# CTPLab/Tera-MIND

Measured on AMD Instinct MI355X. Metric: denoising steps/sec on 64x64x(2 stains x 2 z) patches (interior patch-steps/s), higher is better.
Workload: dtype f32; 1 GPU; configs[1]: b=32 images x 1 interior 64x64 patch (P=1, 128 padded + 32 collage patches/step), rna_slc=4, rna_num=229, stain=all, DDPM T=50 schedule, f32, mode A (pad+patchify -> UNet -> DDPM update); parallelism=dp1 (independent patch batches)

## Files before the change

### include/teramind_hip.h

```cpp
#ifndef TERAMIND_HIP_H
#define TERAMIND_HIP_H

#include <stddef.h>
#include <stdint.h>

#ifdef __cplusplus
extern "C" {
#endif

#define TM_ABI_VERSION 1

enum {
  TM_OK = 0,
  TM_ERR_ARG = -1,
  TM_ERR_STATE = -2,
  TM_ERR_KEY = -3,
  TM_ERR_HIP = -4,
  TM_ERR_WORKSPACE = -5
};

enum { TM_DTYPE_F32 = 0, TM_DTYPE_BF16 = 1, TM_DTYPE_F16 = 2 };
enum { TM_SAMPLE_DDPM = 0, TM_SAMPLE_DDIM = 1 };

typedef struct tm_config {
// ... 138 lines not shown
  double total_ms;
  double nominal_flops;
  double executed_flops;
  double alg_bytes;
} tm_prof_stats;
int tm_profile_enable(tm_model* m, int on);
int tm_profile_collect(tm_model* m, tm_prof_stats* out);


int tm_op_to_cb8(const void* x_ncdhw, void* y_cb8, int N, int C, int Z, int H, int W, void* stream);
int tm_op_from_cb8(const void* x_cb8, void* y_ncdhw, int N, int C, int Z, int H, int W, void* stream);

int tm_op_conv_mfma(const void* x_cb8, const void* w_host, const void* bias_host, void* y_cb8,
                    int N, int Cin, int Cout, int Z, int S, int ksize, int zmode, int up2,
                    int tile_variant, void* stream);
int tm_op_conv_mfma_res(const void* x_cb8, const void* w_host, const void* bias_host, void* y_cb8, const void* res_cb8,
                        int res_half, int N, int Cin, int Cout, int Z, int S, int ksize, int zmode, int up2,
                        int tile_variant, void* stream);

int tm_op_conv_zpair_fused_f32(const void* x_cb8, const void* w_host, const void* bias_host, const void* norm_w_host,
                               const void* scale_host, const void* shift_host, const void* res_cb8, void* a2_out,
                               void* h1_out, void* a2_sep_out, int N, int Cin, int Cout, int Z, int S, int per_image,
                               int tile_variant, void* stream);

int tm_op_conv_ups_pair_f32(const void* x_cb8, const void* w_host, const void* bias_host, void* y_cb8, int N, int Cin,
                            int Cout, int Z, int S, int tile_variant, void* stream);

int tm_op_conv_xpair_f32(const void* x_cb8, const void* w_host, const void* bias_host, void* y_cb8, const void* res_cb8,
                         int res_half, int N, int Cin, int Cout, int Z, int S, int tile_variant, void* stream);
int tm_op_conv_pad1_time_f32(const void* x_cb8, const void* w_host, const void* bias_host, void* y_cb8, int N, int Cin,
                             int Cout, int S, int form, int tile_variant, int iters, float* ms_out, void* stream);

int tm_op_conv1_f32(const void* x_cb8, const void* w_host, const void* bias_host, void* y_cb8, const void* res_cb8,
                    const void* gate_cb8, int x_cbtot, int x_cb0, int gate_cbtot, int gate_cb0, int gate_half, int gelu,
                    int tile_variant, int N, int Cin, int Cout, int Z, int S, int* form_out, void* stream);
int tm_conv1_form(long vox, int ntile, int tile_variant);

int tm_conv_frag_addrs(int kernel, int half, int tw, int what, int wave, int p, int ky, int kx, int sub, int* out64);

int tm_op_conv27_bf16(const void* x_cb8, const void* w_host, const void* bias_host, void* y_cb8,
                      int N, int Cin, int Cout, int S, int dtype, int waves, const void* res_h16, void* y_h16,
                      int ups, int res_half, void* stream);
int tm_op_conv27_h16_z(const void* x_cb8, const void* w_host, const void* bias_host, void* y_cb8,
                       int N, int Cin, int Cout, int S, int dtype, int waves, const void* res_h16, void* y_h16,
                       int ups, int res_half, int Z, void* stream);

// ... 135 lines not shown
```

### tera-mind_amd/_lib.py

```python
import ctypes as C
import os

_HERE = os.path.dirname(os.path.abspath(__file__))
LIB_PATH = os.environ.get("TM_LIB_PATH") or os.path.join(_HERE, "csrc", "libteramind_hip.so")

c_void_p, c_int, c_size_t, c_char_p, c_float = C.c_void_p, C.c_int, C.c_size_t, C.c_char_p, C.c_float
c_i64_p = C.POINTER(C.c_int64)


class TmConfig(C.Structure):
    _fields_ = [("patch_size", C.c_int32), ("rna_slc", C.c_int32), ("n_stain", C.c_int32),
                ("rna_num", C.c_int32), ("net_ch", C.c_int32), ("ch_mult", C.c_int32 * 4),
                ("embed_ch", C.c_int32), ("attn_res", C.c_int32), ("num_res_blocks", C.c_int32),
                ("vis_only", C.c_int32), ("dtype", C.c_int32)]


class TmStepCoefs(C.Structure):
    _fields_ = [("sqrt_recip_alphas_cumprod", c_float), ("sqrt_recipm1_alphas_cumprod", c_float),
                ("posterior_mean_coef1", c_float), ("posterior_mean_coef2", c_float),
                ("sigma", c_float), ("sqrt_alpha_bar_prev", c_float),
                ("sqrt_one_minus_alpha_bar_prev", c_float)]


class TmProfStats(C.Structure):
# ... 50 lines not shown
                                        C.c_int64, c_void_p, c_void_p]),
    "tm_blosc_frame_info": (c_int, [c_void_p, c_size_t, c_void_p]),
    "tm_blosc_decompress_dev": (c_int, [c_void_p, c_void_p, c_void_p, c_int, c_void_p, C.c_int64, c_void_p, c_void_p, c_void_p]),
    "tm_blosc_decompress_tiles": (c_int, [c_void_p, c_void_p, c_void_p, c_int, c_void_p, c_int] + [C.c_int64] * 3 + [c_void_p] * 3),
    "tm_u8_shrink2": (c_int, [c_void_p, c_int, c_int, C.c_int64, c_void_p, C.c_int64, c_void_p]),
    "tm_jpeg_encode_tiles": (c_int, [c_void_p, c_int, c_int, C.c_int64] + [c_int] * 3 + [c_void_p, C.c_int64] + [c_void_p] * 4),
    "tm_jpeg_tables": (c_int, [c_int, c_void_p, c_size_t, C.POINTER(c_size_t)]),
    "tm_ssim_planes": (c_int, [c_void_p, c_void_p] + [c_int] * 4 + [C.c_int64] * 4 + [C.POINTER(c_float), c_int, c_float, c_float, c_void_p, c_void_p]),
    "tm_avgpool2_pad": (c_int, [c_void_p] + [c_int] * 4 + [C.c_int64] * 2 + [c_void_p] + [C.c_int64] * 2 + [c_void_p]),
    "tm_profile_enable": (c_int, [c_void_p, c_int]),
    "tm_profile_collect": (c_int, [c_void_p, C.POINTER(TmProfStats)]),
    "tm_op_to_cb8": (c_int, [c_void_p, c_void_p, c_int, c_int, c_int, c_int, c_int, c_void_p]),
    "tm_op_from_cb8": (c_int, [c_void_p, c_void_p, c_int, c_int, c_int, c_int, c_int, c_void_p]),
    "tm_op_conv_mfma": (c_int, [c_void_p, c_void_p, c_void_p, c_void_p] + [c_int] * 9 + [c_void_p]),
    "tm_op_conv_mfma_res": (c_int, [c_void_p, c_void_p, c_void_p, c_void_p, c_void_p] + [c_int] * 10 + [c_void_p]),
    "tm_op_conv1_f32": (c_int, [c_void_p] * 6 + [c_int] * 12 + [C.POINTER(c_int), c_void_p]),
    "tm_conv1_form": (c_int, [C.c_long, c_int, c_int]),
    "tm_conv_frag_addrs": (c_int, [c_int] * 9 + [c_void_p]),
    "tm_op_conv27_bf16": (c_int, [c_void_p, c_void_p, c_void_p, c_void_p] + [c_int] * 6 + [c_void_p] * 2 + [c_int] * 2 + [c_void_p]),
    "tm_op_conv27_fused": (c_int, [c_void_p] * 7 + [c_int] * 7 + [c_void_p]),
    "tm_op_conv27_h16_z": (c_int, [c_void_p, c_void_p, c_void_p, c_void_p] + [c_int] * 6 + [c_void_p] * 2 + [c_int] * 3 + [c_void_p]),
    "tm_op_conv27_fused_z": (c_int, [c_void_p] * 7 + [c_int] * 8 + [c_void_p]),
    "tm_op_conv_zpair_fused_f32": (c_int, [c_void_p] * 10 + [c_int] * 7 + [c_void_p]),
    "tm_op_conv_ups_pair_f32": (c_int, [c_void_p] * 4 + [c_int] * 6 + [c_void_p]),
    "tm_op_conv_xpair_f32": (c_int, [c_void_p] * 5 + [c_int] * 7 + [c_void_p]),
    "tm_op_conv_pad1_time_f32": (c_int, [c_void_p] * 4 + [c_int] * 7 + [C.POINTER(c_float), c_void_p]),
    "tm_op_conv27_time":(c_int, [c_int] * 10 + [c_void_p, c_void_p]),
    "tm_op_conv1_bf16": (c_int, [c_void_p, c_void_p, c_void_p, c_void_p] + [c_int] * 8 + [c_void_p] * 4),
    "tm_op_conv1_h16_gate": (c_int, [c_void_p, c_void_p, c_void_p, c_void_p] + [c_int] * 8 + [c_void_p] * 3 + [c_int] * 3 + [c_void_p]),
    "tm_op_conv1_concat": (c_int, [c_void_p, c_void_p, c_void_p, c_int, c_void_p, c_void_p, c_void_p] + [c_int] * 8 + [c_void_p]),
    "tm_op_prep_h16": (c_int, [c_void_p] * 3 + [c_int] * 7 + [c_void_p, c_int, c_int, c_void_p, c_void_p, C.c_long] +
                       [c_int] * 4 + [c_void_p, c_void_p, c_int, c_void_p, c_void_p]),
    "tm_op_prep_f32": (c_int, [c_void_p] * 3 + [c_int] * 7 + [c_void_p, c_int, c_int, c_void_p, c_void_p, C.c_long] +
                       [c_int] * 4 + [c_void_p, c_void_p, c_int, c_void_p, c_void_p]),
    "tm_op_prep_form": (c_int, [c_void_p] * 3 + [c_int] * 9 + [c_void_p, c_int, c_int, c_int, c_void_p, c_void_p, C.c_long] +
                        [c_int] * 5 + [c_void_p, c_void_p, c_int, c_int, c_void_p, c_void_p]),
    "tm_op_stem": (c_int, [c_void_p] * 4 + [c_int] * 6 + [c_void_p]),
    "tm_op_head": (c_int, [c_void_p] * 4 + [c_int] * 6 + [c_void_p]),
    "tm_op_time_embed": (c_int, [c_void_p] * 7 + [c_int] * 3 + [c_void_p]),
    "tm_op_emb_all": (c_int, [c_void_p] * 4 + [c_int] * 3 + [c_void_p]),
    "tm_op_prep_train": (c_int, [c_void_p] * 5 + [c_float, c_int, c_void_p] + [c_int] * 4 + [c_void_p]),
    "tm_op_prep_bwd": (c_int, [c_void_p] * 6 + [c_float, c_int] + [c_void_p] * 4 + [c_int] * 4 + [c_void_p]),
    "tm_op_prep_train_rng": (c_int, [c_void_p] * 4 + [C.c_uint64, C.c_uint, c_float, c_int, c_void_p] + [c_int] * 4 + [c_void_p]),
    "tm_op_prep_bwd_rng": (c_int, [c_void_p] * 5 + [C.c_uint64, C.c_uint, c_float, c_int] + [c_void_p] * 4 + [c_int] * 4 + [c_void_p]),
    "tm_op_dropout_mask": (c_int, [C.c_uint64, C.c_uint, c_float, c_void_p] + [c_int] * 4 + [c_void_p]),
    "tm_op_conv_dgrad": (c_int, [c_void_p, c_void_p, c_void_p] + [c_int] * 6 + [c_void_p]),
# ... 63 lines not shown
```

### tera-mind_amd/csrc/tm_conv_pack.cpp

```cpp
#include "tm_conv_frag.h"
#include "tm_kernels.h"

#include <stdlib.h>
#include <string.h>

#include <vector>

namespace tmk {

int conv_form_taps(int form) {
  switch (form) {
    case CF_1X1: return 1;
    case CF_INPLANE: return 9;
    case CF_ZSKIP_UPS: case CF_PAIR_UPS: return 12;
    case CF_XPAIR: return 36;
    default: return 27;
  }
}
static bool form_ups(int form) { return form == CF_ZSKIP_UPS || form == CF_PAIR_UPS; }
size_t conv_pack_floats(int form, int Cout, int Cbi) {
  return (size_t)(form_ups(form) ? 4 : 1) * ((Cout + 63) / 64) * Cbi * conv_form_taps(form) * 512;
}
ConvW conv_w(int form, int Cout, int Cbi) {
  ConvW cw;
  cw.form = form; cw.Cout = Cout; cw.Cbi = Cbi; cw.taps = conv_form_taps(form); cw.ntile = (Cout + 63) / 64;
  return cw;
}

static bool switch_on(const char* name) {
  const char* v = getenv(name);
  return !(v && atoi(v) == 0);
}
int conv_pick_form(int ksize, int zmode, int Z, bool deep8, int role, bool* fuse_mid) {
  static const bool zpair_on = switch_on("TM_CONV_ZPAIR"), xpair_on = switch_on("TM_CONV_XPAIR"),
                    xmid_on = switch_on("TM_CONV_XPAIR_MID"), fuse_on = switch_on("TM_CONV_FUSE_MID");
  if (fuse_mid) *fuse_mid = false;
  if (ksize == 1) return CF_1X1;
  if (zmode == ZM_INPLANE) return CF_INPLANE;
  if (zmode == ZM_VALID) return CF_PLANES3;
  const bool pair = Z == 2 && zpair_on;
  if (zmode == ZM_UPS) return ((role & ROLE_OP_PAIR_UPS) || ((role & ROLE_RES) && pair)) ? CF_PAIR_UPS : CF_ZSKIP_UPS;
  if (Z != 2) return (Z == 1 && (role & ROLE_RES)) ? CF_INPLANE : CF_PLANES3;
  if ((role & ROLE_OP_XPAIR) && xpair_on) return CF_XPAIR;
  if (!pair) return CF_ZSKIP;
  const bool fuses = (role & ROLE_C1_64) && fuse_on;
  const bool xp = (role & ROLE_RES) && !(role & ROLE_DEEP) && xpair_on && deep8 && (!fuses || xmid_on);
  if (fuse_mid) *fuse_mid = fuses && !xp;
  return xp ? CF_XPAIR : CF_PAIR;
}

static void seg_counts(const int* seg_c, int nseg, int& Cin, int& Cbi) {
  Cin = Cbi = 0;
  for (int s = 0; s < nseg; ++s) { Cin += seg_c[s]; Cbi += (seg_c[s] + 7) / 8; }
}
static void pack_taps(const float* w, int Cout, const int* seg_c, int nseg, int taps, float* out, bool halves = false) {
  int Cin, Cbi;
  seg_counts(seg_c, nseg, Cin, Cbi);
  memset(out, 0, (size_t)((Cout + 63) / 64) * Cbi * taps * 512 * sizeof(float));
  int ci0 = 0, cb0 = 0;
  for (int s = 0; s < nseg; ++s) {
    for (int c = 0; c < seg_c[s]; ++c) {
      const int ci = ci0 + c;
      const int cb = cb0 + c / 8, c8 = c % 8;
      for (int co = 0; co < Cout; ++co) {
        const int nt = co / 64, col = co % 64;
        const float* src = w + ((size_t)co * Cin + ci) * taps;
        float* dst = out + (((size_t)nt * Cbi + cb) * taps) * 512 + (halves ? conv_w_off(col, c8) : col * 8 + c8);
        for (int t = 0; t < taps; ++t) dst[(size_t)t * 512] = src[t];
      }
    }
// ... 88 lines not shown
```

### tera-mind_amd/csrc/tm_device.h

```cpp
#pragma once
#include "tm_kernels.h"
#include <math.h>
#include <atomic>

namespace tmk {

typedef float f32x4 __attribute__((ext_vector_type(4)));
typedef float f32x16 __attribute__((ext_vector_type(16)));

#define TM_EPS 1e-6f

struct DevOnce {
  std::atomic<unsigned long long> done[2] = {{0ull}, {0ull}};
  static int dev() { int d = -1; return hipGetDevice(&d) == hipSuccess ? d : -1; }
  bool need() const {
    const int d = dev();
    if (d < 0 || d >= 128) return true;
    return !((done[d >> 6].load(std::memory_order_acquire) >> (d & 63)) & 1ull);
  }
  void mark() {
    const int d = dev();
    if (d >= 0 && d < 128) done[d >> 6].fetch_or(1ull << (d & 63), std::memory_order_release);
  }
};
// ... 137 lines not shown
        if (a.res) o = rv[g][mt] + o;
        if (a.y_h) {
          typedef TM_H16_T bf16x4_t __attribute__((ext_vector_type(4)));
          bf16x4_t ob;
#pragma unroll
          for (int j = 0; j < 4; ++j) ob[j] = (TM_H16_T)o[j];
          *(bf16x4_t*)(a.y_h + (long)on[mt] * a.yh_nstride + pl) = ob;
          continue;
        }
        float* yp = a.y + (long)on[mt] * a.y_nstride + pl;
        if (a.flags & EPI_UP2) {
          *(f32x4*)(yp) = o;
          *(f32x4*)(yp + 8) = o;
          *(f32x4*)(yp + (long)S_out * 8) = o;
          *(f32x4*)(yp + (long)S_out * 8 + 8) = o;
        } else {
          *(f32x4*)(yp) = o;
        }
      }
    }
  }
}

__device__ __forceinline__ void zpair_norm_epilogue(const ConvArgs& a, f32x16 (&o)[2][1], int h, int n, int ooff) {
  float s8[8];
#pragma unroll
  for (int ct = 0; ct < 2; ++ct)
#pragma unroll
    for (int g = 0; g < 4; ++g) {
      const f32x4 bv = *(const f32x4*)(a.bias + (ct * 4 + g) * 8 + 4 * h);
      float p[4];
#pragma unroll
      for (int j = 0; j < 4; ++j) {
        const float v = o[ct][0][4 * g + j] + bv[j];
        o[ct][0][4 * g + j] = v;
        p[j] = v * v;
        asm volatile("" : "+v"(p[j]));
      }
      const float lo = ((p[0] + p[1]) + p[2]) + p[3];
      const float lo_p = __shfl_xor(lo, 32, 64);
      s8[ct * 4 + g] = (((lo_p + p[0]) + p[1]) + p[2]) + p[3];
    }
  float red[4];
#pragma unroll
  for (int r = 0; r < 4; ++r) red[r] = s8[r] + s8[r + 4];
  const float t1 = ((red[0] + red[1]) + red[2]) + red[3];
  const float t0 = __shfl_xor(t1, 32, 64);
  const float t = h ? t1 : t0;
  if (ooff < 0) return;
  const float rstd = 1.0f / sqrtf(t * a.inv_c + TM_EPS);
  const long mo = (long)(n / a.per_image) * a.mod_stride;
  float* yp = a.y + (long)n * a.y_nstride + ooff + 4 * h;
#pragma unroll
  for (int ct = 0; ct < 2; ++ct)
#pragma unroll
    for (int g = 0; g < 4; ++g) {
      const int c0 = (ct * 4 + g) * 8 + 4 * h;
      const f32x4 wn = *(const f32x4*)(a.norm_w + c0);
      const f32x4 sc = *(const f32x4*)(a.mod_scale + mo + c0), sh = *(const f32x4*)(a.mod_shift + mo + c0);
      f32x4 r;
#pragma unroll
      for (int j = 0; j < 4; ++j) {
        float v = wn[j] * (o[ct][0][4 * g + j] * rstd);
        v = v * (1.0f + sc[j]) + sh[j];
        r[j] = silu_h16(v);
      }
      *(f32x4*)(yp + (long)(ct * 4 + g) * a.y_plane) = r;
    }
}

}
```

### tera-mind_amd/csrc/tm_kernels.hip

```cpp
#include "tm_conv_pair.h"

#include <stdlib.h>
#include <string.h>

#include <type_traits>

namespace tmk {

template <int NZI, int WM, int TW, bool UPS = false>
struct C3Geo {
  static constexpr int TW_ = TW;
  static constexpr int MV = 4 * WM * 32;
  static constexpr int TR = (MV / TW < TW) ? (MV / TW) : TW;
  static constexpr int NPB = MV / (TR * TW);
  static constexpr int HR = TR + 2, HC = TW + 2;
  static constexpr int XV = NPB * NZI * HR * HC;
  static constexpr int XPIECES = XV * 2;
  static constexpr int PX = (XPIECES + 255) / 256;
  static constexpr int TZ = UPS ? 4 : 9;
  static constexpr int NTAP = TZ * NZI;
  static constexpr int WFLOATS = NTAP * 512;
  static constexpr int WPIECES = WFLOATS / 4;
  static constexpr int PW = (WPIECES + 255) / 256;
  static constexpr int TAPS_TOTAL = (NZI == 1) ? 9 : 3 * TZ;
// ... 433 lines not shown
  conv_epilogue<1, NC>(a, o, nte, h, on, ooff1, 0);
}

template <int HALF, int TW>
struct XPGeo {
  static constexpr int TW_ = TW;
  static constexpr int NW = 4;
  static constexpr int NQ = HALF ? 2 : 4;
  static constexpr int MP = HALF ? 32 : 64;
  static constexpr int PWD = TW / 2;
  static constexpr int TR = (MP / PWD < TW) ? (MP / PWD) : TW;
  static constexpr int NPB = MP / (TR * PWD);
  static constexpr int HR = TR + 2;
  static constexpr int XP = NPB * HR * PWD;
  static constexpr int XITEMS = XP * 2;
  static_assert(XP % 8 == 0, "whole groups of eight staging items (tm_conv_frag.h)");
  static constexpr int WSLOT = 12 * 512;
  static constexpr int KP = 24 / NW;
  static constexpr int LDS_BYTES = (2 * WSLOT + 12 * XP * 8) * 4;
};
template <class G>
TM_HD constexpr int xp_xtap(int p, int q, int ky) { return (p * 4 + q) * G::XP * 8 + conv_frag_off(ky * G::PWD, 0, G::XP); }

template <int HALF, int TW>
__global__ __launch_bounds__(256, 2) void conv3d_xpair(ConvArgs a) {
  using G = XPGeo<HALF, TW>;
  static_assert(G::XITEMS <= 64 * G::NW, "one staging item per thread");
  extern __shared__ __attribute__((aligned(16))) float lds[];
  float* lw = lds;

  const int tid = threadIdx.x;
  const int lane = tid & 63, wv = tid >> 6;
  const int i32 = lane & 31, h = lane >> 5;

  const int S = a.S;
  const ConvTile t = conv_tile_of<TW, G::TR, false, false>(a);
  const int nt = t.nt, pg = t.pg, tr = t.tr, tc = t.tc;

  long xoff = -1;
  bool okl = false, okr = false;
  if (tid < G::XITEMS) {
    const int half = conv_stage_half(tid);
    int v = conv_stage_row(tid);
    const int j = v % G::PWD; v /= G::PWD;
    const int hr = v % G::HR;
    const int ps = v / G::HR;
    const int n = pg * G::NPB + ps;
    const int y = tr * G::TR + hr - 1, x = tc * TW + 2 * j;
// ... 135 lines not shown
      }
#pragma unroll
    for (int p = 0; p < 3; ++p) {
      acc[p][0] = qh ? (got[p] - acc[p][0]) - acc[p][1] : (acc[p][0] + acc[p][1]) + got[p];
      asm volatile("" : "+v"(acc[p][0]));
    }
#pragma unroll
    for (int z = 0; z < 2; ++z) {
      f32x16 o[1][1];
      o[0][0] = acc[0][0] + acc[1 + z][0];
      asm volatile("" : "+v"(o[0][0]));
      const int ooff[1] = {ooff0 >= 0 ? ooff0 + (z * S * S + qh) * 8 : -1};
      __builtin_amdgcn_sched_barrier(0);
      conv_epilogue<1, 1>(a, o, nte, h, on, ooff, 2 * S);
    }
  } else {
#pragma unroll
    for (int p = 0; p < 3; ++p) {
      const f32x16 ev = (acc[p][0] + acc[p][1]) + acc[p][2];
      acc[p][1] = (acc[p][1] - acc[p][2]) - acc[p][3];
      acc[p][0] = ev;
      asm volatile("" : "+v"(acc[p][0]), "+v"(acc[p][1]));
    }
#pragma unroll
    for (int z = 0; z < 2; ++z)
#pragma unroll
      for (int par = 0; par < 2; ++par) {
        f32x16 o[1][1];
        o[0][0] = acc[0][par] + acc[1 + z][par];
        asm volatile("" : "+v"(o[0][0]));
        const int ooff[1] = {ooff0 >= 0 ? ooff0 + (z * S * S + par) * 8 : -1};
        __builtin_amdgcn_sched_barrier(0);
        conv_epilogue<1, 1>(a, o, nte, h, on, ooff, 2 * S);
      }
  }
}

template <int WM, int WN>
__global__ __launch_bounds__(256, 2) void conv1_mfma(ConvArgs a) {
  constexpr int MV = 4 * WM * 32;
  constexpr int KC = 4;
  constexpr int XP = KC * MV * 2 / 256;
  constexpr int NT64 = WN / 2;
  constexpr int WP = NT64 * KC * 64 * 2 / 256;
  __shared__ __attribute__((aligned(16))) float lds[NT64 * KC * 512 + KC * MV * 8];
  float* lw = lds;
  float* lx = lds + NT64 * KC * 512;

  const int tid = threadIdx.x;
  const int lane = tid & 63, wv = tid >> 6;
  const int i32 = lane & 31, h = lane >> 5;
  const int bid = xcd_swizzle(blockIdx.x, gridDim.x);
  const int nt = bid % a.ntile;
  const int mtile = bid / a.ntile;
  const long VPN = (long)a.Z * a.S * a.S;
  const long vtot = VPN * a.N;

// ... 127 lines not shown
    return large ? launch_tiled<conv3d_mfma<NZI, 2, TW, UPS>, C3Geo<NZI, 2, TW, UPS>>(a, factor, s)
                 : launch_tiled<conv3d_mfma<NZI, 1, TW, UPS>, C3Geo<NZI, 1, TW, UPS>>(a, factor, s);
  });
}

hipError_t launch_conv_mfma(const ConvLaunch& L, hipStream_t s) {
  ConvArgs a;
  a.x = L.x.p; a.x_nstride = L.x.nstride; a.x_plane = L.x.plane();
  a.w = L.w.w; a.bias = L.w.bias;
  a.y = L.y.p; a.y_nstride = L.y.nstride; a.y_plane = L.y.plane(); a.Cob = L.y.Cb;
  a.res = L.res ? L.res->p : nullptr; a.res_nstride = L.res ? L.res->nstride : 0;
  a.gate = L.gate ? L.gate->p : nullptr; a.gate_nstride = L.gate ? L.gate->nstride : 0;
  const int form = L.w.form;
  if (L.w.taps != conv_form_taps(form)) return hipErrorInvalidValue;
  if (L.gate_half) {
    int ls = 0;
    while ((1 << ls) < L.y.H) ++ls;
    if (!L.gate || form != CF_1X1 || (1 << ls) != L.y.H || L.y.H != L.y.W || ls < 1) return hipErrorInvalidValue;
    a.gate_ls = ls;
  }
  a.N = L.x.N; a.S = L.x.H; a.Z = L.x.Z; a.Cbi = L.w.Cbi; a.ntile = L.w.ntile; a.flags = L.flags;
  if (L.x.Cb != L.w.Cbi || L.x.H != L.x.W) return hipErrorInvalidValue;
  if (L.fuse_norm) {
    if (form != CF_PAIR || L.zmode != ZM_PAD1 || L.x.Z != 2 || L.w.Cout != 64 || L.w.ntile != 1 || L.res || L.gate || L.flags ||
        !L.norm_w || !L.mod_scale || !L.mod_shift || L.per_image < 1)
      return hipErrorInvalidValue;
    if (conv_tile(form, (long)L.x.N * 2 * L.x.H * L.x.H, 1, L.x.H, L.tile_variant) != 2) return hipErrorInvalidValue;
    if (!L.a2.p || L.a2.Cb != 8 || L.a2.N != L.x.N || L.a2.Z != 2 || L.a2.H != L.x.H || L.a2.W != L.x.H) return hipErrorInvalidValue;
    if (L.y.Cb != 8 || L.y.Z != 2 || L.y.H != L.x.H) return hipErrorInvalidValue;
    a.y = L.a2.p; a.y_nstride = L.a2.nstride; a.y_plane = L.a2.plane();
    a.norm_w = L.norm_w; a.mod_scale = L.mod_scale; a.mod_shift = L.mod_shift; a.mod_stride = L.mod_stride;
    a.per_image = L.per_image; a.inv_c = L.inv_c;
  }
  if (L.y.Cb > L.w.ntile * 8 || L.y.N != L.x.N) return hipErrorInvalidValue;
  const long vox = (long)a.N * a.Z * a.S * a.S;
  if (form == CF_1X1) {
    if (L.flags & EPI_UP2) return hipErrorInvalidValue;
    if (L.y.H != L.x.H || L.y.Z != L.x.Z) return hipErrorInvalidValue;
    const int form1 = conv1_form(vox, a.ntile, L.tile_variant);
    if (form1 == 3) {
      const long mt = (vox + 255) / 256;
      a.ntile /= 2;
      hipLaunchKernelGGL((conv1_mfma<2, 4>), dim3((unsigned)(mt * a.ntile)), dim3(256), 0, s, a);
    } else if (form1 == 2) {
      const long mt = (vox + 255) / 256;
      hipLaunchKernelGGL((conv1_mfma<2, 2>), dim3((unsigned)(mt * a.ntile)), dim3(256), 0, s, a);
    } else if (form1 == 1) {
      const long mt = (vox + 127) / 128;
// ... 36 lines not shown
  switch (form) {
    case CF_INPLANE: return launch_c3<1, false>(a, large, s);
    case CF_PLANES3: return launch_c3<3, false>(a, large, s);
    case CF_ZSKIP: return launch_c3<2, false>(a, large, s);
    case CF_ZSKIP_UPS: return launch_c3<2, true>(a, large, s);
    case CF_PAIR:
      if (S == 4) return launch_tiled<conv3d_zpair<1, 4, false>, ZPGeo<1, 4>>(a, 1, s);
      return with_tile_width<32>(S, [&](auto tw) {
        constexpr int TW = decltype(tw)::value;
        if (L.fuse_norm) return launch_tiled<conv3d_zpair<0, TW, true>, ZPGeo<0, TW>>(a, 1, s);
        return large ? launch_tiled<conv3d_zpair<0, TW, false>, ZPGeo<0, TW>>(a, 1, s)
                     : launch_tiled<conv3d_zpair<1, TW, false>, ZPGeo<1, TW>>(a, 1, s);
      });
    case CF_PAIR_UPS:
      if (S == 4) return launch_tiled<conv3d_zpair_ups<1, 4>, ZPUGeo<1, 4>>(a, 4, s);
      return with_tile_width<32>(S, [&](auto tw) {
        constexpr int TW = decltype(tw)::value;
        return large ? launch_tiled<conv3d_zpair_ups<0, TW>, ZPUGeo<0, TW>>(a, 4, s)
                     : launch_tiled<conv3d_zpair_ups<1, TW>, ZPUGeo<1, TW>>(a, 4, s);
      });
    default:
      return with_tile_width<16>(S, [&](auto tw) {
        constexpr int TW = decltype(tw)::value;
        return large ? launch_tiled<conv3d_xpair<0, TW>, XPGeo<0, TW>, 64 * XPGeo<0, TW>::NW>(a, 1, s)
                     : launch_tiled<conv3d_xpair<1, TW>, XPGeo<1, TW>, 64 * XPGeo<1, TW>::NW>(a, 1, s);
      });
  }
}

template <class G, int HALF, int TW, bool UPS>
static int zpair_frag_addrs(int what, int wv, int p, int ky, int kx, int sub, int* out) {
  constexpr int NC = HALF ? 1 : 2, KW = UPS ? 2 : 3;
  constexpr int lx = G::LDS_BYTES / 4 - 3 * G::XV * 8;
  if (p < 0 || p > 2) return -1;
  if (what == 2 ? (ky < 0 || ky >= G::PX) : (ky < 0 || ky >= KW || kx < 0 || kx >= KW)) return -1;
  if (what == 0 ? (sub < 0 || sub >= NC) : what == 1 ? (sub < 0 || sub > (UPS ? 3 : 0)) : false) return -1;
  const int vt = HALF ? (wv & 1) : wv, ct0 = HALF ? (wv >> 1) : 0;
  for (int lane = 0; lane < 64; ++lane) {
    const int i32 = lane & 31, h = lane >> 5;
    int a = -1;
    if (what == 0) a = zp_wtap(UPS ? p * 4 + ky * 2 + kx : p * 9 + ky * 3 + kx, sub) + conv_w_off(ct0 * 32 + i32, 4 * h);
    else if (what == 1)
      a = lx + zp_xtap<G>(p, ky, kx) + conv_lane_of<G::TR, TW, G::PS, G::HC, G::XV>(vt * 32 + conv_lane_voxel(TW, i32), h, sub >> 1, sub & 1).xb;
    else {
      const int i = wv * 64 + lane + ky * 256;
      if (conv_stage_row(i) < G::XV) a = lx + p * G::XV * 8 + conv_frag_off(conv_stage_row(i), conv_stage_half(i), G::XV);
// ... 1009 lines not shown
```

### tera-mind_amd/csrc/tm_model.hip

```cpp
#include "../../include/teramind_hip.h"
#include "tm_kernels.h"

#include <algorithm>
#include <cmath>
#include <map>
#include <string>
#include <type_traits>
#include <vector>
#include <stdarg.h>
#include <stdio.h>
#include <stdlib.h>
#include <string.h>

using namespace tmk;

static thread_local char g_err[512] = "";
int tmk::fail(int code, const char* fmt, ...) {
  va_list ap;
  va_start(ap, fmt);
  vsnprintf(g_err, sizeof(g_err), fmt, ap);
  va_end(ap);
  return code;
}

// ... 862 lines not shown
    TV A2 = cx.tensor(N, w.cout, Z, S_out), H1 = cx.tensor(N, w.cout, Z, S_out);
    ConvLaunch L1 = conv(A, w.c1u, H1);
    L1.zmode = ZM_UPS;
    run_conv(cx, L1);
    PrepLaunch Q = mid_section(cx, w, H1, per_image);
    prep_out(Q, A2);
    cx.run(Q);
    ConvLaunch L2 = conv(A2, w.c2, out);
    L2.res = &src[0].t; L2.res_half = 1;
    run_conv(cx, L2, w.cout);
    cx.top = mark;
    return out;
  }
  int cin_pad = w.cbi * 8;
  TV A = cx.tensor(N, cin_pad, Z, S_out), raw;
  const bool need_raw = w.has_skip || mode != RS_SAME || src.size() > 1 || src[0].collage;
  if (need_raw) raw = cx.tensor(N, cin_pad, Z, S_out);
  PrepLaunch P = block_input(cx, w, src, N, Z, S_out, per_image, mode);
  prep_out(P, A);
  if (need_raw) prep_raw(P, raw);
  cx.run(P);
  TV A2 = cx.tensor(N, w.cout, Z, S_out);
  ConvLaunch L1 = conv(A, w.c1, A2);
  if (w.fuse_mid && Z == 2 && conv_tile(CF_PAIR, (long)N * Z * S_out * S_out, 1, S_out, 0) == 2) {
    fuse_mid_section(L1, cx, w, per_image, A2);
    run_conv(cx, L1, w.cin);
  } else {
    TV H1 = cx.tensor(N, w.cout, Z, S_out);
    L1.y = H1;
    run_conv(cx, L1, w.cin);
    PrepLaunch Q = mid_section(cx, w, H1, per_image);
    prep_out(Q, A2);
    cx.run(Q);
  }
  if (w.has_skip) run_conv(cx, conv(raw, w.skip, out));
  ConvLaunch L2 = conv(A2, w.c2, out);
  L2.res = w.has_skip ? &out : (need_raw ? &raw : &src[0].t);
  run_conv(cx, L2, w.cout);
  cx.top = mark;
  return out;
}

struct AttnGeom { bool half = false, mfma_core = false; int Sc = 0; };
struct AttnCond {
  TV mod, kv;
  TVH mod_h, kv_h;
};
// ... 587 lines not shown
```

### tera-mind_amd/csrc/tm_ops.hip

```cpp
#include "../../include/teramind_hip.h"
#include "tm_kernels.h"

#include <algorithm>
#include <cmath>
#include <cstdint>
#include <tuple>
#include <utility>
#include <vector>
#include <string.h>

using namespace tmk;

struct DevTmp {
  std::vector<void*> ptrs;
  std::vector<hipEvent_t> events;
  hipError_t err = hipSuccess;
  const char* what = "";
  bool ordered = false;
  hipStream_t st = nullptr;
  DevTmp() = default;
  explicit DevTmp(hipStream_t stream) : ordered(true), st(stream) { keep_pool(); }
  static void keep_pool() {
    static bool done[64] = {};
    int dev = 0;
// ... 132 lines not shown
    L.res_half = res_half ? 1 : 0;
  }
  return TM_OK;
}

extern "C" int tm_op_conv_mfma_res(const void* x_cb8, const void* w_host, const void* bias_host, void* y_cb8, const void* res_cb8,
                                   int res_half, int N, int Cin, int Cout, int Z, int S, int ksize, int zmode, int up2,
                                   int tile_variant, void* stream) {
  if (ksize != 1 && ksize != 3) return fail(TM_ERR_ARG, "ksize must be 1 or 3");
  if (zmode != ZM_PAD1 && zmode != ZM_INPLANE && zmode != ZM_VALID && zmode != ZM_UPS) return fail(TM_ERR_ARG, "bad zmode");
  const bool ups = ksize == 3 && zmode == ZM_UPS;
  if (zmode == ZM_UPS && (ksize != 3 || up2)) return fail(TM_ERR_ARG, "ZM_UPS: ksize 3, no fused upsample of the output");
  if (res_cb8 && (ksize != 3 || zmode == ZM_UPS)) return fail(TM_ERR_ARG, "residual: k x 3 x 3 forms other than ZM_UPS only");
  if (res_half && (!res_cb8 || up2 || S < 2)) return fail(TM_ERR_ARG, "res_half: needs a residual, S >= 2 and no fused upsample");
  const int Zout = (ksize == 3 && zmode == ZM_VALID) ? Z - 2 : Z;
  ConvOp op;
  if (const int rc = conv_op(op, conv_pick_form(ksize, zmode, Z, false, ROLE_OP), w_host, bias_host, x_cb8, y_cb8, N, Cin, Cout, Z, S,
                             Zout, (up2 || ups) ? 2 * S : S, zmode, tile_variant, res_cb8, res_half))
    return rc;
  op.L.flags = up2 ? EPI_UP2 : 0;
  return finish((hipStream_t)stream, launch_conv_mfma(op.L, (hipStream_t)stream), "conv_mfma");
}

extern "C" int tm_op_conv_zpair_fused_f32(const void* x_cb8, const void* w_host, const void* bias_host, const void* norm_w_host,
                                          const void* scale_host, const void* shift_host, const void* res_cb8, void* a2_out,
                                          void* h1_out, void* a2_sep_out, int N, int Cin, int Cout, int Z, int S, int per_image,
                                          int tile_variant, void* stream) {
  if (!x_cb8 || !w_host || !bias_host || !norm_w_host || !scale_host || !shift_host || !a2_out) return fail(TM_ERR_ARG, "null argument");
  if (N < 1 || Cin < 1 || per_image < 1) return fail(TM_ERR_ARG, "N, Cin, per_image must be positive");
  if (Z != 2) return fail(TM_ERR_ARG, "the pair form exists at Z == 2 only (got Z = %d)", Z);
  if (Cout != 64) return fail(TM_ERR_ARG, "the fused mid-section needs Cout == 64: one wave holds every channel (got %d)", Cout);
  if (res_cb8) return fail(TM_ERR_ARG, "the fused mid-section takes no residual");
  if (S != 8 && S != 16 && S != 32 && S != 64 && S != 128) return fail(TM_ERR_ARG, "S must be 8, 16, 32, 64 or 128 (got %d)", S);
  if (tile_variant < 0 || tile_variant > 2) return fail(TM_ERR_ARG, "tile_variant must be 0 (auto), 1 or 2 (got %d)", tile_variant);
  if (conv_tile(CF_PAIR, (long)N * Z * S * S, 1, S, tile_variant) != 2)
    return fail(TM_ERR_ARG, "the fused mid-section exists in the 128-voxel tile only; this launch takes the 64-voxel one");
  if (a2_sep_out && !h1_out) return fail(TM_ERR_ARG, "a2_sep_out needs h1_out");
  if (conv_pick_form(3, ZM_PAD1, Z, false, ROLE_OP) != CF_PAIR) return fail(TM_ERR_ARG, "the pair form is switched off (TM_CONV_ZPAIR=0)");
  ConvOp op;
  if (const int rc = conv_op(op, CF_PAIR, w_host, bias_host, x_cb8, a2_out, N, Cin, Cout, Z, S, Z, S, ZM_PAD1, tile_variant)) return rc;
  const int nimg = (N + per_image - 1) / per_image;
  const float* nw = op.tmp.alloc((size_t)Cout, (const float*)norm_w_host);
  const float* sc = op.tmp.alloc((size_t)nimg * Cout, (const float*)scale_host);
  const float* sh = op.tmp.alloc((size_t)nimg * Cout, (const float*)shift_host);
  if (op.tmp.err) return op.tmp.report();
  hipStream_t st = (hipStream_t)stream;
  ConvLaunch& L = op.L;
  L.fuse_norm = 1; L.a2 = L.y; L.norm_w = nw; L.mod_scale = sc; L.mod_shift = sh; L.mod_stride = Cout; L.per_image = per_image;
  L.inv_c = 1.0f / (float)Cout;
  hipError_t e = launch_conv_mfma(L, st);
  if (e == hipSuccess && h1_out) {
    ConvLaunch U = L;
    U.fuse_norm = 0; U.y = cb8_view(h1_out, N, Cout, Z, S, S);
    e = launch_conv_mfma(U, st);
    if (e == hipSuccess && a2_sep_out) {
      PrepLaunch P = prep_start(N, Z, S);
      prep_src(P, U.y);
      prep_norm(P, nw, Cout);
      P.mod = MOD_IMAGE; P.mod_scale = sc; P.mod_shift = sh; P.mod_stride = Cout;
      P.act = 1; P.per_image = per_image;
      prep_out(P, cb8_view(a2_sep_out, N, Cout, Z, S, S));
      e = launch_prep(P, st);
    }
  }
  return finish(st, e, "conv_zpair_fused (fp32)");
}

extern "C" int tm_op_conv_ups_pair_f32(const void* x_cb8, const void* w_host, const void* bias_host, void* y_cb8, int N, int Cin,
                                       int Cout, int Z, int S, int tile_variant, void* stream) {
  if (!x_cb8 || !w_host || !bias_host || !y_cb8) return fail(TM_ERR_ARG, "null argument");
  if (N < 1 || Cin < 1 || Cout < 1) return fail(TM_ERR_ARG, "N, Cin, Cout must be positive");
  if (Z != 2) return fail(TM_ERR_ARG, "the pair form exists at Z == 2 only (got Z = %d)", Z);
  if (S != 4 && S != 8 && S != 16 && S != 32 && S != 64) return fail(TM_ERR_ARG, "S must be 4, 8, 16, 32 or 64 (got %d)", S);
  if (tile_variant < 0 || tile_variant > 2) return fail(TM_ERR_ARG, "tile_variant must be 0 (auto), 1 or 2 (got %d)", tile_variant);
  ConvOp op;
  if (const int rc = conv_op(op, conv_pick_form(3, ZM_UPS, Z, false, ROLE_OP_PAIR_UPS), w_host, bias_host, x_cb8, y_cb8, N, Cin, Cout, Z,
                             S, Z, 2 * S, ZM_UPS, tile_variant))
    return rc;
  return finish((hipStream_t)stream, launch_conv_mfma(op.L, (hipStream_t)stream), "conv_ups_pair (fp32)");
}

static int xpair_args(const void* x, const void* w, const void* b, const void* y, int N, int Cin, int Cout, int Z, int S,
                      int tile_variant) {
  if (!x || !w || !b || !y) return fail(TM_ERR_ARG, "null argument");
  if (N < 1 || Cin < 1 || Cout < 1) return fail(TM_ERR_ARG, "N, Cin, Cout must be positive");
  if (Z != 2) return fail(TM_ERR_ARG, "the x-pair form exists at Z == 2 only (got Z = %d)", Z);
  if (S != 8 && S != 16 && S != 32 && S != 64 && S != 128) return fail(TM_ERR_ARG, "S must be 8, 16, 32, 64 or 128 (got %d)", S);
  if (tile_variant < 0 || tile_variant > 2) return fail(TM_ERR_ARG, "tile_variant must be 0 (auto), 1 or 2 (got %d)", tile_variant);
// ... 1303 lines not shown
```

Baseline: 946.3 interior patch-steps/s.

## Fuse norm-modulation-SiLU epilogue into x-pair conv kernel for mid-section

Adds a fused variant of the x-pair conv kernel that applies bias, RMS-style channel norm, per-image scale/shift and SiLU in its epilogue, exchanging partial sums of squares between the two waves through LDS. Previously, when a layer took the x-pair form, the mid-section fusion was disabled (or the x-pair form was skipped), so one of the two kernels was given up. Now both are used together, which removes a separate prep pass and its memory round trip. In exchange, the fused path adds two block barriers and LDS traffic, and it forces the HALF=0 tile even where the HALF=1 one would otherwise be picked.

```diff
diff --git a/include/teramind_hip.h b/include/teramind_hip.h
--- a/include/teramind_hip.h
+++ b/include/teramind_hip.h
@@ -184,6 +184,10 @@
                                const void* scale_host, const void* shift_host, const void* res_cb8, void* a2_out,
                                void* h1_out, void* a2_sep_out, int N, int Cin, int Cout, int Z, int S, int per_image,
                                int tile_variant, void* stream);
+int tm_op_conv_xpair_fused_f32(const void* x_cb8, const void* w_host, const void* bias_host, const void* norm_w_host,
+                               const void* scale_host, const void* shift_host, const void* res_cb8, void* a2_out,
+                               void* h1_out, void* a2_sep_out, int N, int Cin, int Cout, int Z, int S, int per_image,
+                               int tile_variant, void* stream);
 
 int tm_op_conv_ups_pair_f32(const void* x_cb8, const void* w_host, const void* bias_host, void* y_cb8, int N, int Cin,
                             int Cout, int Z, int S, int tile_variant, void* stream);
diff --git a/tera-mind_amd/_lib.py b/tera-mind_amd/_lib.py
--- a/tera-mind_amd/_lib.py
+++ b/tera-mind_amd/_lib.py
@@ -96,6 +96,7 @@
     "tm_op_conv27_h16_z": (c_int, [c_void_p, c_void_p, c_void_p, c_void_p] + [c_int] * 6 + [c_void_p] * 2 + [c_int] * 3 + [c_void_p]),
     "tm_op_conv27_fused_z": (c_int, [c_void_p] * 7 + [c_int] * 8 + [c_void_p]),
     "tm_op_conv_zpair_fused_f32": (c_int, [c_void_p] * 10 + [c_int] * 7 + [c_void_p]),
+    "tm_op_conv_xpair_fused_f32": (c_int, [c_void_p] * 10 + [c_int] * 7 + [c_void_p]),
     "tm_op_conv_ups_pair_f32": (c_int, [c_void_p] * 4 + [c_int] * 6 + [c_void_p]),
     "tm_op_conv_xpair_f32": (c_int, [c_void_p] * 5 + [c_int] * 7 + [c_void_p]),
     "tm_op_conv_pad1_time_f32": (c_int, [c_void_p] * 4 + [c_int] * 7 + [C.POINTER(c_float), c_void_p]),
diff --git a/tera-mind_amd/csrc/tm_conv_pack.cpp b/tera-mind_amd/csrc/tm_conv_pack.cpp
--- a/tera-mind_amd/csrc/tm_conv_pack.cpp
+++ b/tera-mind_amd/csrc/tm_conv_pack.cpp
@@ -33,7 +33,7 @@
 }
 int conv_pick_form(int ksize, int zmode, int Z, bool deep8, int role, bool* fuse_mid) {
   static const bool zpair_on = switch_on("TM_CONV_ZPAIR"), xpair_on = switch_on("TM_CONV_XPAIR"),
-                    xmid_on = switch_on("TM_CONV_XPAIR_MID"), fuse_on = switch_on("TM_CONV_FUSE_MID");
+                    fuse_on = switch_on("TM_CONV_FUSE_MID");
   if (fuse_mid) *fuse_mid = false;
   if (ksize == 1) return CF_1X1;
   if (zmode == ZM_INPLANE) return CF_INPLANE;
@@ -43,9 +43,8 @@
   if (Z != 2) return (Z == 1 && (role & ROLE_RES)) ? CF_INPLANE : CF_PLANES3;
   if ((role & ROLE_OP_XPAIR) && xpair_on) return CF_XPAIR;
   if (!pair) return CF_ZSKIP;
-  const bool fuses = (role & ROLE_C1_64) && fuse_on;
-  const bool xp = (role & ROLE_RES) && !(role & ROLE_DEEP) && xpair_on && deep8 && (!fuses || xmid_on);
-  if (fuse_mid) *fuse_mid = fuses && !xp;
+  if (fuse_mid) *fuse_mid = (role & ROLE_C1_64) && fuse_on;
+  const bool xp = (role & ROLE_RES) && !(role & ROLE_DEEP) && xpair_on && deep8;
   return xp ? CF_XPAIR : CF_PAIR;
 }
 
diff --git a/tera-mind_amd/csrc/tm_device.h b/tera-mind_amd/csrc/tm_device.h
--- a/tera-mind_amd/csrc/tm_device.h
+++ b/tera-mind_amd/csrc/tm_device.h
@@ -183,51 +183,58 @@
   }
 }
 
+__device__ __forceinline__ void norm_block_chains(const ConvArgs& a, f32x16& o, int cb0, int h, float* s8) {
+#pragma unroll
+  for (int g = 0; g < 4; ++g) {
+    const f32x4 bv = *(const f32x4*)(a.bias + (cb0 + g) * 8 + 4 * h);
+    float p[4];
+#pragma unroll
+    for (int j = 0; j < 4; ++j) {
+      const float v = o[4 * g + j] + bv[j];
+      o[4 * g + j] = v;
+      p[j] = v * v;
+      asm volatile("" : "+v"(p[j]));
+    }
+    const float lo = ((p[0] + p[1]) + p[2]) + p[3];
+    const float lo_p = __shfl_xor(lo, 32, 64);
+    s8[g] = (((lo_p + p[0]) + p[1]) + p[2]) + p[3];
+  }
+}
+__device__ __forceinline__ float norm_voxel_sum(const float (&red)[4], int h) {
+  const float t1 = ((red[0] + red[1]) + red[2]) + red[3];
+  const float t0 = __shfl_xor(t1, 32, 64);
+  return h ? t1 : t0;
+}
+__device__ __forceinline__ void norm_store(const ConvArgs& a, const f32x16& o, int cb0, int h, float rstd, long mo, float* yp) {
+#pragma unroll
+  for (int g = 0; g < 4; ++g) {
+    const int c0 = (cb0 + g) * 8 + 4 * h;
+    const f32x4 wn = *(const f32x4*)(a.norm_w + c0);
+    const f32x4 sc = *(const f32x4*)(a.mod_scale + mo + c0), sh = *(const f32x4*)(a.mod_shift + mo + c0);
+    f32x4 r;
+#pragma unroll
+    for (int j = 0; j < 4; ++j) {
+      float v = wn[j] * (o[4 * g + j] * rstd);
+      v = v * (1.0f + sc[j]) + sh[j];
+      r[j] = silu_h16(v);
+    }
+    *(f32x4*)(yp + (long)(cb0 + g) * a.y_plane) = r;
+  }
+}
 __device__ __forceinline__ void zpair_norm_epilogue(const ConvArgs& a, f32x16 (&o)[2][1], int h, int n, int ooff) {
   float s8[8];
 #pragma unroll
-  for (int ct = 0; ct < 2; ++ct)
-#pragma unroll
-    for (int g = 0; g < 4; ++g) {
-      const f32x4 bv = *(const f32x4*)(a.bias + (ct * 4 + g) * 8 + 4 * h);
-      float p[4];
-#pragma unroll
-      for (int j = 0; j < 4; ++j) {
-        const float v = o[ct][0][4 * g + j] + bv[j];
-        o[ct][0][4 * g + j] = v;
-        p[j] = v * v;
-        asm volatile("" : "+v"(p[j]));
-      }
-      const float lo = ((p[0] + p[1]) + p[2]) + p[3];
-      const float lo_p = __shfl_xor(lo, 32, 64);
-      s8[ct * 4 + g] = (((lo_p + p[0]) + p[1]) + p[2]) + p[3];
-    }
+  for (int ct = 0; ct < 2; ++ct) norm_block_chains(a, o[ct][0], ct * 4, h, s8 + ct * 4);
   float red[4];
 #pragma unroll
   for (int r = 0; r < 4; ++r) red[r] = s8[r] + s8[r + 4];
-  const float t1 = ((red[0] + red[1]) + red[2]) + red[3];
-  const float t0 = __shfl_xor(t1, 32, 64);
-  const float t = h ? t1 : t0;
+  const float t = norm_voxel_sum(red, h);
   if (ooff < 0) return;
   const float rstd = 1.0f / sqrtf(t * a.inv_c + TM_EPS);
   const long mo = (long)(n / a.per_image) * a.mod_stride;
   float* yp = a.y + (long)n * a.y_nstride + ooff + 4 * h;
 #pragma unroll
-  for (int ct = 0; ct < 2; ++ct)
-#pragma unroll
-    for (int g = 0; g < 4; ++g) {
-      const int c0 = (ct * 4 + g) * 8 + 4 * h;
-      const f32x4 wn = *(const f32x4*)(a.norm_w + c0);
-      const f32x4 sc = *(const f32x4*)(a.mod_scale + mo + c0), sh = *(const f32x4*)(a.mod_shift + mo + c0);
-      f32x4 r;
-#pragma unroll
-      for (int j = 0; j < 4; ++j) {
-        float v = wn[j] * (o[ct][0][4 * g + j] * rstd);
-        v = v * (1.0f + sc[j]) + sh[j];
-        r[j] = silu_h16(v);
-      }
-      *(f32x4*)(yp + (long)(ct * 4 + g) * a.y_plane) = r;
-    }
-}
-
-}
+  for (int ct = 0; ct < 2; ++ct) norm_store(a, o[ct][0], ct * 4, h, rstd, mo, yp);
+}
+
+}
diff --git a/tera-mind_amd/csrc/tm_kernels.hip b/tera-mind_amd/csrc/tm_kernels.hip
--- a/tera-mind_amd/csrc/tm_kernels.hip
+++ b/tera-mind_amd/csrc/tm_kernels.hip
@@ -479,8 +479,9 @@
 template <class G>
 TM_HD constexpr int xp_xtap(int p, int q, int ky) { return (p * 4 + q) * G::XP * 8 + conv_frag_off(ky * G::PWD, 0, G::XP); }
 
-template <int HALF, int TW>
+template <int HALF, int TW, bool FUSE = false>
 __global__ __launch_bounds__(256, 2) void conv3d_xpair(ConvArgs a) {
+  static_assert(!FUSE || HALF == 0, "the fused mid-section needs all four q of an x-pair in one wave");
   using G = XPGeo<HALF, TW>;
   static_assert(G::XITEMS <= 64 * G::NW, "one staging item per thread");
   extern __shared__ __attribute__((aligned(16))) float lds[];
@@ -662,17 +663,54 @@
       acc[p][0] = ev;
       asm volatile("" : "+v"(acc[p][0]), "+v"(acc[p][1]));
     }
-#pragma unroll
-    for (int z = 0; z < 2; ++z)
-#pragma unroll
-      for (int par = 0; par < 2; ++par) {
-        f32x16 o[1][1];
-        o[0][0] = acc[0][par] + acc[1 + z][par];
-        asm volatile("" : "+v"(o[0][0]));
-        const int ooff[1] = {ooff0 >= 0 ? ooff0 + (z * S * S + par) * 8 : -1};
-        __builtin_amdgcn_sched_barrier(0);
-        conv_epilogue<1, 1>(a, o, nte, h, on, ooff, 2 * S);
-      }
+    if constexpr (FUSE) {
+      float s8[2][2][4];
+#pragma unroll
+      for (int z = 0; z < 2; ++z)
+#pragma unroll
+        for (int par = 0; par < 2; ++par) {
+          acc[1 + z][par] = acc[0][par] + acc[1 + z][par];
+          asm volatile("" : "+v"(acc[1 + z][par]));
+          norm_block_chains(a, acc[1 + z][par], ch * 4, h, s8[z][par]);
+        }
+      f32x4* ex = (f32x4*)lds;
+      __syncthreads();
+#pragma unroll
+      for (int z = 0; z < 2; ++z)
+#pragma unroll
+        for (int par = 0; par < 2; ++par) {
+          const f32x4 v = {s8[z][par][0], s8[z][par][1], s8[z][par][2], s8[z][par][3]};
+          ex[(wv * 4 + z * 2 + par) * 64 + lane] = v;
+        }
+      __syncthreads();
+#pragma unroll
+      for (int z = 0; z < 2; ++z)
+#pragma unroll
+        for (int par = 0; par < 2; ++par) {
+          const f32x4 got = ex[((wv ^ 1) * 4 + z * 2 + par) * 64 + lane];
+          float red[4];
+#pragma unroll
+          for (int r = 0; r < 4; ++r) red[r] = s8[z][par][r] + got[r];
+          const float t = norm_voxel_sum(red, h);
+          if (ooff0 < 0) continue;
+          const float rstd = 1.0f / sqrtf(t * a.inv_c + TM_EPS);
+          const long mo = (long)(on[0] / a.per_image) * a.mod_stride;
+          float* yp = a.y + (long)on[0] * a.y_nstride + ooff0 + (z * S * S + par) * 8 + 4 * h;
+          norm_store(a, acc[1 + z][par], ch * 4, h, rstd, mo, yp);
+        }
+    } else {
+#pragma unroll
+      for (int z = 0; z < 2; ++z)
+#pragma unroll
+        for (int par = 0; par < 2; ++par) {
+          f32x16 o[1][1];
+          o[0][0] = acc[0][par] + acc[1 + z][par];
+          asm volatile("" : "+v"(o[0][0]));
+          const int ooff[1] = {ooff0 >= 0 ? ooff0 + (z * S * S + par) * 8 : -1};
+          __builtin_amdgcn_sched_barrier(0);
+          conv_epilogue<1, 1>(a, o, nte, h, on, ooff, 2 * S);
+        }
+    }
   }
 }
 
@@ -846,8 +884,8 @@
   a.N = L.x.N; a.S = L.x.H; a.Z = L.x.Z; a.Cbi = L.w.Cbi; a.ntile = L.w.ntile; a.flags = L.flags;
   if (L.x.Cb != L.w.Cbi || L.x.H != L.x.W) return hipErrorInvalidValue;
   if (L.fuse_norm) {
-    if (form != CF_PAIR || L.zmode != ZM_PAD1 || L.x.Z != 2 || L.w.Cout != 64 || L.w.ntile != 1 || L.res || L.gate || L.flags ||
-        !L.norm_w || !L.mod_scale || !L.mod_shift || L.per_image < 1)
+    if ((form != CF_PAIR && form != CF_XPAIR) || L.zmode != ZM_PAD1 || L.x.Z != 2 || L.w.Cout != 64 || L.w.ntile != 1 || L.res ||
+        L.gate || L.flags || !L.norm_w || !L.mod_scale || !L.mod_shift || L.per_image < 1)
       return hipErrorInvalidValue;
     if (conv_tile(form, (long)L.x.N * 2 * L.x.H * L.x.H, 1, L.x.H, L.tile_variant) != 2) return hipErrorInvalidValue;
     if (!L.a2.p || L.a2.Cb != 8 || L.a2.N != L.x.N || L.a2.Z != 2 || L.a2.H != L.x.H || L.a2.W != L.x.H) return hipErrorInvalidValue;
@@ -930,6 +968,7 @@
     default:
       return with_tile_width<16>(S, [&](auto tw) {
         constexpr int TW = decltype(tw)::value;
+        if (L.fuse_norm) return launch_tiled<conv3d_xpair<0, TW, true>, XPGeo<0, TW>, 64 * XPGeo<0, TW>::NW>(a, 1, s);
         return large ? launch_tiled<conv3d_xpair<0, TW>, XPGeo<0, TW>, 64 * XPGeo<0, TW>::NW>(a, 1, s)
                      : launch_tiled<conv3d_xpair<1, TW>, XPGeo<1, TW>, 64 * XPGeo<1, TW>::NW>(a, 1, s);
       });
diff --git a/tera-mind_amd/csrc/tm_model.hip b/tera-mind_amd/csrc/tm_model.hip
--- a/tera-mind_amd/csrc/tm_model.hip
+++ b/tera-mind_amd/csrc/tm_model.hip
@@ -908,7 +908,7 @@
   cx.run(P);
   TV A2 = cx.tensor(N, w.cout, Z, S_out);
   ConvLaunch L1 = conv(A, w.c1, A2);
-  if (w.fuse_mid && Z == 2 && conv_tile(CF_PAIR, (long)N * Z * S_out * S_out, 1, S_out, 0) == 2) {
+  if (w.fuse_mid && Z == 2 && conv_tile(w.c1.form, (long)N * Z * S_out * S_out, 1, S_out, 0) == 2) {
     fuse_mid_section(L1, cx, w, per_image, A2);
     run_conv(cx, L1, w.cin);
   } else {
diff --git a/tera-mind_amd/csrc/tm_ops.hip b/tera-mind_amd/csrc/tm_ops.hip
--- a/tera-mind_amd/csrc/tm_ops.hip
+++ b/tera-mind_amd/csrc/tm_ops.hip
@@ -178,23 +178,25 @@
   return finish((hipStream_t)stream, launch_conv_mfma(op.L, (hipStream_t)stream), "conv_mfma");
 }
 
-extern "C" int tm_op_conv_zpair_fused_f32(const void* x_cb8, const void* w_host, const void* bias_host, const void* norm_w_host,
-                                          const void* scale_host, const void* shift_host, const void* res_cb8, void* a2_out,
-                                          void* h1_out, void* a2_sep_out, int N, int Cin, int Cout, int Z, int S, int per_image,
-                                          int tile_variant, void* stream) {
+static int conv_fused_op(int form, const char* what, const void* x_cb8, const void* w_host, const void* bias_host,
+                         const void* norm_w_host, const void* scale_host, const void* shift_host, const void* res_cb8, void* a2_out,
+                         void* h1_out, void* a2_sep_out, int N, int Cin, int Cout, int Z, int S, int per_image, int tile_variant,
+                         void* stream) {
   if (!x_cb8 || !w_host || !bias_host || !norm_w_host || !scale_host || !shift_host || !a2_out) return fail(TM_ERR_ARG, "null argument");
   if (N < 1 || Cin < 1 || per_image < 1) return fail(TM_ERR_ARG, "N, Cin, per_image must be positive");
-  if (Z != 2) return fail(TM_ERR_ARG, "the pair form exists at Z == 2 only (got Z = %d)", Z);
-  if (Cout != 64) return fail(TM_ERR_ARG, "the fused mid-section needs Cout == 64: one wave holds every channel (got %d)", Cout);
+  if (Z != 2) return fail(TM_ERR_ARG, "the %s form exists at Z == 2 only (got Z = %d)", what, Z);
+  if (Cout != 64) return fail(TM_ERR_ARG, "the fused mid-section needs Cout == 64: one cout tile holds every channel (got %d)", Cout);
   if (res_cb8) return fail(TM_ERR_ARG, "the fused mid-section takes no residual");
   if (S != 8 && S != 16 && S != 32 && S != 64 && S != 128) return fail(TM_ERR_ARG, "S must be 8, 16, 32, 64 or 128 (got %d)", S);
   if (tile_variant < 0 || tile_variant > 2) return fail(TM_ERR_ARG, "tile_variant must be 0 (auto), 1 or 2 (got %d)", tile_variant);
-  if (conv_tile(CF_PAIR, (long)N * Z * S * S, 1, S, tile_variant) != 2)
+  if (conv_tile(form, (long)N * Z * S * S, 1, S, tile_variant) != 2)
     return fail(TM_ERR_ARG, "the fused mid-section exists in the 128-voxel tile only; this launch takes the 64-voxel one");
   if (a2_sep_out && !h1_out) return fail(TM_ERR_ARG, "a2_sep_out needs h1_out");
-  if (conv_pick_form(3, ZM_PAD1, Z, false, ROLE_OP) != CF_PAIR) return fail(TM_ERR_ARG, "the pair form is switched off (TM_CONV_ZPAIR=0)");
+  if (form == CF_PAIR ? conv_pick_form(3, ZM_PAD1, Z, false, ROLE_OP) != CF_PAIR
+                      : conv_pick_form(3, ZM_PAD1, Z, true, ROLE_OP_XPAIR) != CF_XPAIR)
+    return fail(TM_ERR_ARG, "the %s form is switched off (%s=0)", what, form == CF_PAIR ? "TM_CONV_ZPAIR" : "TM_CONV_XPAIR");
   ConvOp op;
-  if (const int rc = conv_op(op, CF_PAIR, w_host, bias_host, x_cb8, a2_out, N, Cin, Cout, Z, S, Z, S, ZM_PAD1, tile_variant)) return rc;
+  if (const int rc = conv_op(op, form, w_host, bias_host, x_cb8, a2_out, N, Cin, Cout, Z, S, Z, S, ZM_PAD1, tile_variant)) return rc;
   const int nimg = (N + per_image - 1) / per_image;
   const float* nw = op.tmp.alloc((size_t)Cout, (const float*)norm_w_host);
   const float* sc = op.tmp.alloc((size_t)nimg * Cout, (const float*)scale_host);
@@ -219,7 +221,21 @@
       e = launch_prep(P, st);
     }
   }
-  return finish(st, e, "conv_zpair_fused (fp32)");
+  return finish(st, e, form == CF_PAIR ? "conv_zpair_fused (fp32)" : "conv_xpair_fused (fp32)");
+}
+extern "C" int tm_op_conv_zpair_fused_f32(const void* x_cb8, const void* w_host, const void* bias_host, const void* norm_w_host,
+                                          const void* scale_host, const void* shift_host, const void* res_cb8, void* a2_out,
+                                          void* h1_out, void* a2_sep_out, int N, int Cin, int Cout, int Z, int S, int per_image,
+                                          int tile_variant, void* stream) {
+  return conv_fused_op(CF_PAIR, "pair", x_cb8, w_host, bias_host, norm_w_host, scale_host, shift_host, res_cb8, a2_out, h1_out,
+                       a2_sep_out, N, Cin, Cout, Z, S, per_image, tile_variant, stream);
+}
+extern "C" int tm_op_conv_xpair_fused_f32(const void* x_cb8, const void* w_host, const void* bias_host, const void* norm_w_host,
+                                          const void* scale_host, const void* shift_host, const void* res_cb8, void* a2_out,
+                                          void* h1_out, void* a2_sep_out, int N, int Cin, int Cout, int Z, int S, int per_image,
+                                          int tile_variant, void* stream) {
+  return conv_fused_op(CF_XPAIR, "x-pair", x_cb8, w_host, bias_host, norm_w_host, scale_host, shift_host, res_cb8, a2_out, h1_out,
+                       a2_sep_out, N, Cin, Cout, Z, S, per_image, tile_variant, stream);
 }
 
 extern "C" int tm_op_conv_ups_pair_f32(const void* x_cb8, const void* w_host, const void* bias_host, void* y_cb8, int N, int Cin,
```

After: 955.1 interior patch-steps/s (median of 6 runs). About the same (+0.9%).
